# NVIDIA/flownet2-pytorch

Hardware: AMD Instinct MI355X
Metric: image-pairs/sec, FlowNet2 custom-layer hot path (Correlation + Resample2d + ChannelNorm) fwd+bwd @ 384x512 bs8 -- the whole FlowNet2C network's fwd+bwd image-pairs/sec is flownet2c.fwd_bwd_image_pairs_per_s; corr-layer HBM GB/s vs roofline is `roofline` (higher is better)
Workload: dtype f32; 1 GPU; FlowNet2 custom-layer hot path fwd+bwd, bs8 @384x512: Correlation 8x256x48x64 (20,1,20,1,2) [BASELINE configs[1]] + Resample2d 8x3x384x512 + ChannelNorm 8x3x384x512

## Files before the change

flownet2-pytorch_amd/csrc/corr_params.h:

```cpp
#pragma once
#include "fn2_common.h"

namespace fn2 {

struct CorrP {
    int B, C, H, W;
    int pad, k, md, s1, s2;
    int kr, dr, D, nOut, oH, oW;
    long out_bs;
    float slope;
};

int corr_make_params(CorrP &p, int B, int C, int H, int W, int pad, int k, int md, int s1, int s2);
int corr_forward_direct(const void *in1, const void *in2, void *out, int dtype, const CorrP &p, hipStream_t s);
int corr_backward_direct(const void *in1, const void *in2, const void *gout, void *g1, void *g2, int dtype,
                         const CorrP &p, hipStream_t s);

bool corr_dense_applicable(int dtype, int C, int H, int W, int pad, int k, int md, int s1, int s2);
bool corr_dense_forward_pays(const CorrP &p);
int corr_forward_dense(const void *in1, const void *in2, void *out, int dtype, const CorrP &p, hipStream_t s);
int corr_backward_dense(const void *in1, const void *in2, const void *gout, void *g1, void *g2, int dtype,
                        const CorrP &p, hipStream_t s);
bool corr_mfma_f32_applicable(int dtype, int C, int H, int W, int pad, int k, int md, int s1, int s2);
int corr_forward_mfma_f32(const float *in1, const float *in2, float *out, long out_bs, float slope, int B, int C, int H,
                          int W, int md, int tune, hipStream_t s);

bool corr_f16x2_applicable(int dtype, int C, int H, int W, int pad, int k, int md, int s1, int s2);
int corr_forward_f16x2(const float *in1, const float *in2, float *out, long out_bs, float slope, int B, int C, int H, int W,
                       int variant, hipStream_t s);
int corr_forward_f16x2_wide(const float *in1, const float *in2, float *out, long out_bs, float slope, int B, int C, int H, int W,
                            hipStream_t s);

bool corr_f16_fwd_applicable(int dtype, int C, int H, int W, int pad, int k, int md, int s1, int s2);
int corr_forward_f16(int dtype, const void *in1, const void *in2, void *out, long out_bs, float slope, int B, int C, int H, int W,
                     hipStream_t s);

bool corr_f16_bwd_applicable(int dtype, int C, int H, int W, int pad, int k, int md, int s1, int s2);
int corr_backward_f16(int dtype, const void *in1, const void *in2, const void *gout, void *g1, void *g2, int B, int C, int H, int W,
                      hipStream_t s);

void corr_f16x2_set_debug_buffer(void *p);
void *corr_f16x2_get_debug_buffer();
bool corr_bwd_f16x2_applicable(int dtype, int C, int H, int W, int pad, int k, int md, int s1, int s2);
int corr_backward_f16x2(const float *in1, const float *in2, const float *gout, float *g1, float *g2, int B, int C, int H, int W,
                        int variant, hipStream_t s);
int corr_backward_f16x2_wide(const float *in1, const float *in2, const float *gout, float *g1, float *g2, int B, int C, int H, int W,
                             hipStream_t s);

bool corr_bwd_mfma_f32_applicable(int dtype, int C, int H, int W, int pad, int k, int md, int s1, int s2);
int corr_backward_mfma_f32(const float *in1, const float *in2, const float *gout, float *g1, float *g2,
                           int B, int C, int H, int W, int md, int tune, hipStream_t s);

bool corr_mfma_f64_applicable(int dtype, int C, int H, int W, int pad, int k, int md, int s1, int s2);
int corr_forward_mfma_f64(const double *in1, const double *in2, double *out, long out_bs, double slope, int B, int C, int H, int W, hipStream_t s);
int corr_backward_mfma_f64(const double *in1, const double *in2, const double *gout, double *g1, double *g2, int B, int C, int H, int W, hipStream_t s);

}
```

flownet2-pytorch_amd/csrc/correlation_f16_bwd.hip:

```cpp
#include <type_traits>

#include "corr_params.h"

#ifndef FN2_HBH_ABL
#define FN2_HBH_ABL 0
#endif

namespace fn2 {
namespace hbh {
constexpr int ABL = FN2_HBH_ABL;

typedef float f4 __attribute__((ext_vector_type(4)));
typedef unsigned u4 __attribute__((ext_vector_type(4)));
typedef unsigned u2 __attribute__((ext_vector_type(2)));
#define FN2_LDS(T) __attribute__((address_space(3))) T

constexpr int DR = 10, D = 21, NU = 6;
constexpr int CG = 64, NCT = CG / 16;
constexpr int CK = 32;
constexpr int CHS = 288, PARS = CK * CHS, XBUF = 2 * PARS;
template <int FLIP> struct GL {
    static constexpr int BI = 256;
    static constexpr int TI = FLIP ? 1024 + 4 : 1024 + 32;
    static constexpr int AI = FLIP ? D * TI + 76 : D * TI + 128;
// ... 61 lines not shown
struct XSet { u4 v[XK]; };
struct GSet { u4 v[NGL]; };

template <class E>
__global__ __launch_bounds__(NWAVES * 64, 3) void corr_bwd_f16(Args<E> p)
{
    typedef typename Op16<E>::v8 h8;
    __shared__ __attribute__((aligned(16))) char smem[LDS_BYTES];

    const int tid = threadIdx.x, lane = tid & 63;
    const int wave = __builtin_amdgcn_readfirstlane(tid >> 6);
    const bool is_stage = wave < NSW;
    const int w8 = is_stage ? wave : wave - NSW;
    const int HL = p.H >> 1;
    const int hw = p.H * p.W;
    const long HW = (long)p.H * p.W;
    const int per_fn = 2 * p.NRG * p.NCGR;
    const int ntasks = 2 * p.B * per_fn;
    const bool pow2 = (p.C & (p.C - 1)) == 0;

    struct Task { int flip, n, py, rg, cg; };
    auto get_task = [&](int t) -> Task {
        Task k;
        k.cg = t % p.NCGR; t /= p.NCGR;
        k.rg = t % p.NRG; t /= p.NRG;
        k.py = t & 1; t >>= 1;
        k.n = t % p.B;
        k.flip = t / p.B;
        k.cg = __builtin_amdgcn_readfirstlane(k.cg); k.rg = __builtin_amdgcn_readfirstlane(k.rg);
        k.py = __builtin_amdgcn_readfirstlane(k.py); k.n = __builtin_amdgcn_readfirstlane(k.n);
        k.flip = __builtin_amdgcn_readfirstlane(k.flip);
        return k;
    };

    float *Es = reinterpret_cast<float *>(smem + X_OFS);
    auto store_rows = [&](const Task &tk) {
        if (ABL & 32) return;
        int ln = lane;
        asm volatile("" : "+v"(ln));
        const int g = ln >> 4, xg = 4 * (ln & 15);
        constexpr int NRI = (CG + NWAVES - 1) / NWAVES;
        const int y = 2 * (4 * tk.rg + g) + tk.py;
        const bool lane_ok = 4 * tk.rg + g < HL && xg < p.W;
        const unsigned vo = lane_ok ? (unsigned)((y * p.W + xg) * 2) : 0x80000000u;
        const __amdgpu_buffer_rsrc_t rso = __builtin_amdgcn_make_buffer_rsrc(p.gin[tk.flip] + (long)tk.n * p.C * HW, 0, (unsigned)(p.C * hw * 2), 0x00020000);
        auto chan = [&](int i) { return wave + NWAVES * i; };
        auto read_row = [&](int c) {
            return *reinterpret_cast<const f4 *>(Es + (c * 4 + g) * 64 + ((xg + 8 * g + 32 * ((c >> 2) & 1)) & 63));
        };
        f4 vals[NRI];
#pragma unroll
        for (int i = 0; i < NRI; ++i) vals[i] = read_row(chan(i) & (CG - 1));
        float r, f = 1.0f;
        asm volatile("v_mov_b32 %0, %1" : "=v"(r) : "s"(p.rC));
        if (!pow2) asm volatile("v_mov_b32 %0, %1" : "=v"(f) : "s"(p.fC));
        auto finish = [&](f4 val) -> u2 {
            if (pow2) { val[0] *= r; val[1] *= r; val[2] *= r; val[3] *= r; }
            else { val[0] /= f; val[1] /= f; val[2] /= f; val[3] /= f; }
            return (u2){Op16<E>::pk(val[0], val[1]), Op16<E>::pk(val[2], val[3])};
        };
        unsigned bad = 0;
#pragma unroll
        for (int i = 0; i < NRI; ++i) {
            const int c = chan(i);
            if (c >= CG) continue;
            if (lane_ok && (__builtin_amdgcn_classf(vals[i][0], 0x207) | __builtin_amdgcn_classf(vals[i][1], 0x207) |
// ... 73 lines not shown
            asm volatile("" : "+v"(ln));
            const int ts = ln >> 3, pc = ln & 7;
            if (tk.flip) {
                char *dst = smem + w8 * GL<1>::AI + ts * GL<1>::TI + pc * 32;
#pragma unroll
                for (int i = 0; i < NGL; ++i) {
                    const int bi = i / 3, tb = i % 3;
                    if (tb == 2 && ts + 16 >= D) continue;
                    const h8 h = __builtin_bit_cast(h8, S.v[i]);
                    FN2_LDS(float) *d = (FN2_LDS(float) *)(dst + 8 * tb * GL<1>::TI + bi * 256);
#pragma unroll
                    for (int e = 0; e < 8; ++e) d[e] = (float)h[e];
                }
            } else {
                char *dst = smem + w8 * GL<0>::AI + ts * GL<0>::TI + pc * 32;
#pragma unroll
                for (int i = 0; i < NGL; ++i) {
                    const int bi = i / 3, tb = i % 3;
                    if (tb == 2 && ts + 16 >= D) continue;
                    const h8 h = __builtin_bit_cast(h8, S.v[i]);
                    *(FN2_LDS(f4) *)(dst + 8 * tb * GL<0>::TI + bi * 256) = (f4){(float)h[0], (float)h[1], (float)h[2], (float)h[3]};
                    *(FN2_LDS(f4) *)(dst + 8 * tb * GL<0>::TI + bi * 256 + 16) = (f4){(float)h[4], (float)h[5], (float)h[6], (float)h[7]};
                }
            }
        };
        auto pick = [](bool c, const Task &a, const Task &b) {
            Task r;
            r.flip = c ? a.flip : b.flip; r.n = c ? a.n : b.n; r.py = c ? a.py : b.py; r.rg = c ? a.rg : b.rg; r.cg = c ? a.cg : b.cg;
            return r;
        };
        XSet XA0, XA1, XB0, XB1;
        GSet GS;
        int t = (int)xcd_remap(blockIdx.x, gridDim.x);
        if (t < ntasks) {
            const Task tk = get_task(t);
            g_issue(GS, tk, 0, true);
            x_issue(XA0, tk, 0, 0, true);
            x_issue(XA1, tk, 0, 1, true);
            g_write(GS, tk);
            g_issue(GS, tk, 1, true);
        }
        __syncthreads();
        for (; t < ntasks; t += gridDim.x) {
            const Task tk = get_task(t);
            const bool has_next = t + (int)gridDim.x < ntasks;
            const Task tn = get_task(has_next ? t + (int)gridDim.x : t);
            auto one_u = [&](int u, XSet &C0, XSet &C1, XSet &N0, XSet &N1) {
                const bool more = u + 1 < NU, more2 = u + 2 < NU;
                const Task t1 = pick(more, tk, tn), t2 = pick(more2, tk, tn);
                x_issue(N0, t1, more ? u + 1 : 0, 0, more || has_next);
                x_issue(N1, t1, more ? u + 1 : 0, 1, more || has_next);
                x_write(C0, smem + X_OFS);
                x_write(C1, smem + X_OFS + XBUF);
                __syncthreads();
                if (more || has_next) g_write(GS, t1);
                g_issue(GS, t2, more2 ? u + 2 : u + 2 - NU, more2 || has_next);
                __syncthreads();
            };
            for (int u = 0; u < NU; u += 2) {
                one_u(u, XA0, XA1, XB0, XB1);
                one_u(u + 1, XB0, XB1, XA0, XA1);
            }
            __syncthreads();
            store_rows(tk);
            __syncthreads();
        }
        return;
    }

    const int xpar = w8 & 1;
    const int role = __builtin_amdgcn_readfirstlane(w8 >> 1);

    auto run_task = [&](const Task &tk, auto flipc) {
        constexpr int FLIP = decltype(flipc)::value;
        int ln = lane;
        asm volatile("" : "+v"(ln));
        const int f_i = ln & 15, f_g = ln >> 4;
        const int f_ai = f_i >> 2, f_aj = f_i & 3;
        const int xb = xpar * PARS + f_i * CHS + f_g * 16;

        f4 acc[2][NCT];
#pragma unroll
        for (int ab = 0; ab < 2; ++ab)
#pragma unroll
            for (int ct = 0; ct < NCT; ++ct) acc[ab][ct] = (f4){0.0f, 0.0f, 0.0f, 0.0f};
        h8 gh[NF];

        auto gather = [&](auto role_c, auto xp_c) {
            constexpr int R = decltype(role_c)::value;
            constexpr int XP = decltype(xp_c)::value;
            typedef GL<FLIP> L;
            constexpr int SB = L::TI - 8;
            int l2 = lane;
            asm volatile("" : "+v"(l2));
// ... 46 lines not shown
#pragma unroll
                    for (int ct = 0; ct < NCT; ++ct)
                        x[ct] = *reinterpret_cast<const h8 *>(smem + X_OFS + (ct >> 1) * XBUF + xb + (ct & 1) * 16 * CHS + j * 64);
                    if (ABL & 1) { asm volatile("" ::"v"(x[0]), "v"(x[1]), "v"(x[2]), "v"(x[3])); return; }
#pragma unroll
                    for (int ct = 0; ct < NCT; ++ct) {
                        if constexpr (f0 >= 0) acc[0][ct] = Op16<E>::mfma(x[ct], gh[f0 >= 0 ? f0 : 0], acc[0][ct]);
                        if constexpr (f1 >= 0) acc[1][ct] = Op16<E>::mfma(x[ct], gh[f1 >= 0 ? f1 : 0], acc[1][ct]);
                    }
                    __builtin_amdgcn_sched_barrier(0);
                }
            });
        };
        auto gather_d = [&]() {
            auto by_role = [&](auto xp_c) {
                switch (role) {
                case 0: gather(std::integral_constant<int, 0>{}, xp_c); break;
                case 1: gather(std::integral_constant<int, 1>{}, xp_c); break;
                case 2: gather(std::integral_constant<int, 2>{}, xp_c); break;
                default: gather(std::integral_constant<int, 3>{}, xp_c); break;
                }
            };
            if (xpar) by_role(std::integral_constant<int, 1>{});
            else by_role(std::integral_constant<int, 0>{});
        };
        auto mma_d = [&]() {
            switch (role) {
            case 0: mma(std::integral_constant<int, 0>{}); break;
            case 1: mma(std::integral_constant<int, 1>{}); break;
            case 2: mma(std::integral_constant<int, 2>{}); break;
            default: mma(std::integral_constant<int, 3>{}); break;
            }
        };
        for (int u = 0; u < NU; ++u) {
            gather_d();
            __syncthreads();
            mma_d();
            __syncthreads();
        }
        auto scatter = [&](auto role_c) {
            constexpr int R = decltype(role_c)::value;
            static_for<0, 2>([&](auto abc) {
                constexpr int ab = decltype(abc)::value;
                constexpr int a = a_blk(R, ab);
                const int x = 8 * a + 2 * f_aj + xpar;
                static_for<0, NCT>([&](auto ctc) {
                    constexpr int ct = decltype(ctc)::value;
                    static_for<0, 4>([&](auto rc) {
                        constexpr int r = decltype(rc)::value;
                        const int c = 16 * ct + 4 * f_g + r;
                        Es[(c * 4 + f_ai) * 64 + ((x + 8 * f_ai + 32 * (f_g & 1)) & 63)] = acc[ab][ct][r];
                    });
                });
            });
        };
        if (ABL & 32) {
#pragma unroll
            for (int ab = 0; ab < 2; ++ab)
#pragma unroll
                for (int ct = 0; ct < NCT; ++ct) asm volatile("" ::"v"(acc[ab][ct]));
        } else {
            switch (role) {
            case 0: scatter(std::integral_constant<int, 0>{}); break;
            case 1: scatter(std::integral_constant<int, 1>{}); break;
            case 2: scatter(std::integral_constant<int, 2>{}); break;
            default: scatter(std::integral_constant<int, 3>{}); break;
            }
// ... 52 lines not shown
```

flownet2-pytorch_amd/csrc/correlation_f16x2_bwd.hip:

```cpp
#include <type_traits>

#include "corr_params.h"
#include "f16x2_split.h"

namespace fn2 {
namespace hb {
using f16s::exp_stat;
using f16s::scale_exp;
using f16s::split2;
using f16s::to_sgpr;
using f16s::wave_sum;

typedef float f4 __attribute__((ext_vector_type(4)));
typedef float f2 __attribute__((ext_vector_type(2)));
typedef _Float16 h2 __attribute__((ext_vector_type(2)));
typedef _Float16 h8 __attribute__((ext_vector_type(8)));
typedef short s8 __attribute__((ext_vector_type(8)));
typedef unsigned u4 __attribute__((ext_vector_type(4)));
typedef unsigned u2 __attribute__((ext_vector_type(2)));
#define FN2_LDS(T) __attribute__((address_space(3))) T

#ifdef FN2_ABL_BWDTEMPORAL
constexpr int BWD_STORE_AUX = 0;
#else
// ... 93 lines not shown
    asm volatile("v_mbcnt_lo_u32_b32 %0, -1, 0\n\tv_mbcnt_hi_u32_b32 %0, -1, %0" : "=v"(l));
    return l;
}

template <int VAR>
__global__ __launch_bounds__(NWAVES * 64, 3) void corr_bwd_f16x2(Args p)
{
    __shared__ __attribute__((aligned(16))) char smem[LDS_BYTES];
    __shared__ int scl_k[2];
    __shared__ __attribute__((aligned(16))) float scl_sx[2][CG];

    const int tid = threadIdx.x, lane = tid & 63;
    const int wave = __builtin_amdgcn_readfirstlane(tid >> 6);
    const bool is_stage = wave < NSW;
    const int w8 = is_stage ? wave : wave - NSW;
    const int HL = p.H >> 1;
    const long HW = (long)p.H * p.W;
    const int per_fn = 2 * p.NRG * p.NCGR;
    const int ntasks = p.nflip * p.B * per_fn;
    const bool pow2 = (p.C & (p.C - 1)) == 0;
    const int lgC = pow2 ? 31 - __builtin_clz((unsigned)p.C) : 0;
    if (tid < 16) reinterpret_cast<unsigned *>(smem + ZERO_OFS)[tid] = 0u;
    unsigned long long ts[16];
#pragma unroll
    for (int i = 0; i < 16; ++i) ts[i] = 0;
    auto stamp = [&](int i) __attribute__((always_inline)) { if (VAR & 64) ts[i] = __builtin_amdgcn_s_memtime(); };
    auto dump = [&]() __attribute__((always_inline)) {
        if ((VAR & 64) && p.dbg && lane == 0 && (wave == 0 || wave == NSW)) {
            unsigned long long *d = p.dbg + (blockIdx.x * 2 + (wave ? 1 : 0)) * 16;
#pragma unroll
            for (int i = 0; i < 16; ++i) d[i] = ts[i];
        }
    };
    stamp(0);

    struct Task { int flip, n, py, rg, cg; };
    auto get_task = [&](int t) -> Task {
        Task k;
        k.cg = t % p.NCGR; t /= p.NCGR;
        k.rg = t % p.NRG; t /= p.NRG;
#ifdef FN2_ABL_FLIPOUTER
        k.py = t & 1; t >>= 1;
        k.n = t % p.B;
        k.flip = p.nflip == 2 ? t / p.B : p.flip0;
#else
        k.flip = p.nflip == 2 ? t % 2 : p.flip0;
        if (p.nflip == 2) t >>= 1;
        k.py = t & 1; t >>= 1;
        k.n = t;
#endif
        k.cg = __builtin_amdgcn_readfirstlane(k.cg); k.rg = __builtin_amdgcn_readfirstlane(k.rg);
        k.py = __builtin_amdgcn_readfirstlane(k.py); k.n = __builtin_amdgcn_readfirstlane(k.n);
        k.flip = __builtin_amdgcn_readfirstlane(k.flip);
        return k;
    };

    float *Es = reinterpret_cast<float *>(smem + X_OFS);
    auto store_rows = [&](const Task &tk, int kg, int par) {
        int ln = lane_now();
        const int g = ln >> 4, xg = 4 * (ln & 15);
        constexpr int NRI = (CG + NWAVES - 1) / NWAVES;
        const int y = 2 * (4 * tk.rg + g) + tk.py;
        const bool lane_ok = 4 * tk.rg + g < HL && xg < p.W;
        const unsigned vo = lane_ok ? (unsigned)((y * p.W + xg) * 4) : 0x80000000u;
        const __amdgpu_buffer_rsrc_t rso = __builtin_amdgcn_make_buffer_rsrc(p.gin[tk.flip] + (long)tk.n * p.C * HW, 0, (unsigned)(p.C * HW * 4), 0x00020000);
        auto chan = [&](int i) { return wave + NWAVES * i; };
        auto read_row = [&](int c) {
            return *reinterpret_cast<const f4 *>(Es + (c * 4 + g) * 64 + ((xg + 8 * g + 32 * ((c >> 2) & 1)) & 63));
        };
        f4 vals[NRI];
#pragma unroll
        for (int i = 0; i < NRI; ++i) vals[i] = read_row(chan(i) & (CG - 1));
        float f = 1.0f;
        if (!pow2) asm volatile("v_mov_b32 %0, %1" : "=v"(f) : "s"(p.fC));
        const int kx_ex = -lgC;
        auto ksum_of = [&](int c) {
            const int cc = c & (CG - 1);
            const int bits = to_sgpr(__builtin_bit_cast(int, scl_sx[par][8 * (cc & 7) + (cc >> 3)]));
            return (bits >> 23) - 127 + kg;
        };
        auto scaled = [&](f4 val, int kx) {
#pragma unroll
            for (int e = 0; e < 4; ++e) val[e] = __builtin_ldexpf(val[e], kx);
            if (!pow2) { val[0] /= f; val[1] /= f; val[2] /= f; val[3] /= f; }
            return val;
        };
        unsigned bad = 0;
// ... 101 lines not shown
            const int tj = tk.flip ? 20 - 4 * U0 - bi + ai : 4 * U0 + bi - ai;
            const int ilg = tk.flip ? 4 * tk.rg - DR + 4 * U0 + bi : 4 * tk.rg + ai;
            const int x = 2 * (((((5 * ln) >> 1) & 31) * (p.W >> 1)) >> 5);
            const int c = tk.cg * CG + ln, ilx = min(4 * tk.rg + (ln & 3), HL - 1);
            const int ti = (5 * q + (ln & 3) + bi) % D;
            const unsigned ox = (ilx >= 0 && ilx < HL) ? (unsigned)((c * HW + (long)(2 * ilx + tk.py) * p.W + x) * 4) : 0x80000000u;
            const int ilx2 = min(4 * tk.rg + ((ln + 2) & 3), HL - 1), xb = (x + (p.W >> 1)) >= p.W ? x + (p.W >> 1) - p.W : x + (p.W >> 1);
            const unsigned ox2 = (ilx2 >= 0 && ilx2 < HL) ? (unsigned)((c * HW + (long)(2 * ilx2 + tk.py) * p.W + xb) * 4) : 0x80000000u;
            const unsigned og = (ilg >= 0 && ilg < HL) ? (unsigned)((((tj * D + ti) * p.H + 2 * ilg + tk.py) * p.W + x) * 4) : 0x80000000u;
#ifdef FN2_ABL_NOSAMPLELOAD
            S.x = (u2)0x3f000000u; S.x2 = S.x; S.g = (u2)0x3f000000u; (void)ox; (void)ox2; (void)og;
#else
            S.x = (VAR & 2) ? (u2)0x3f800000u : __builtin_amdgcn_raw_buffer_load_b64(rsx, (int)ox, 0, 0);
            S.x2 = (VAR & 2) ? (u2)0x3f800000u : __builtin_amdgcn_raw_buffer_load_b64(rsx, (int)ox2, 0, 0);
            S.g = (VAR & 2) ? (u2)0x3f800000u : __builtin_amdgcn_raw_buffer_load_b64(rsg, (int)og, 0, 0);
#endif
        };
        auto sample_scales = [&](const Samp &S, int &kx, int &kg) {
            const unsigned t4 = exp_stat(S.x[0]) + exp_stat(S.x[1]) + exp_stat(S.x2[0]) + exp_stat(S.x2[1]);
            const unsigned sum = t4 & 0xffffu, cnt = t4 >> 16;
            const int em = cnt ? (int)((2u * sum + cnt) / (2u * cnt)) : 0;
            const int k = f16s::T_GEO + 127 - em;
            kx = cnt == 0u ? 0 : (k < -126 ? -126 : k > 127 ? 127 : k);
            const unsigned tg = exp_stat(S.g[0]) + exp_stat(S.g[1]);
            kg = scale_exp(wave_sum(tg));
        };
        auto publish = [&](int par, int kx, int kg) {
            if (wave == 0) {
                int ln = lane_now();
                scl_sx[par][8 * (ln & 7) + (ln >> 3)] = f16s::scale_from_exp(kx);
                if (ln == 0) scl_k[1] = kg;
            }
        };
        XSet XA0, XA1, XB0, XB1;
        int t = (int)xcd_remap(blockIdx.x, gridDim.x);
        Samp SM;
        int kx_n = 0, kg_n = 0;
        int it = 0;
        if (t < ntasks) {
            const Task tk = get_task(t);
            sample_issue(tk, SM);
            x_issue(XA0, tk, 0, 0);
            x_issue(XA1, tk, 0, 1);
            g_dma(tk, 0);
            stamp(1);
            dma_wait();
            stamp(2);
            sample_scales(SM, kx_n, kg_n);
            publish(0, kx_n, kg_n);
        }
        __syncthreads();
        stamp(3);
        for (; t < ntasks; t += gridDim.x) {
            const Task tk = get_task(t);
            const bool has_next = t + (int)gridDim.x < ntasks;
            const Task tn = get_task(has_next ? t + (int)gridDim.x : t);
            const bool first = t < (int)gridDim.x;
            const int kg_cur = kg_n, par = it & 1;
            auto one_u = [&](int u, XSet &C0, XSet &C1, XSet &N0, XSet &N1) {
                const float *sxp = &scl_sx[par][8 * s_ch];
                float sc = sxp[0];
                if (u + 1 < NU) { x_issue(N0, tk, u + 1, 0); x_issue(N1, tk, u + 1, 1); }
                else if (has_next) { x_issue(N0, tn, 0, 0); x_issue(N1, tn, 0, 1); }
#pragma unroll
                for (int k = 0; k < 2 * XK; ++k) {
                    const float nx = sxp[k + 1 < 2 * XK ? k + 1 : k];
                    if (k < XK) x_write1(C0, smem + X_OFS, k, sc);
                    else x_write1(C1, smem + X_OFS + XBUF, k - XK, sc);
                    sc = nx;
                }
                if (first && u < 2) stamp(4 + 4 * u);
                __syncthreads();
                if (first && u < 2) stamp(5 + 4 * u);
                if (u + 1 < NU) g_dma(tk, u + 1);
                else if (has_next) { sample_issue(tn, SM); g_dma(tn, 0); }
                dma_wait();
                if (first && u < 2) stamp(6 + 4 * u);
                __syncthreads();
                if (first && u < 2) stamp(7 + 4 * u);
            };
            for (int u = 0; u < NU; u += 2) {
                one_u(u, XA0, XA1, XB0, XB1);
                one_u(u + 1, XB0, XB1, XA0, XA1);
            }
            if (has_next) { sample_scales(SM, kx_n, kg_n); publish(par ^ 1, kx_n, kg_n); }
            if (first) stamp(12);
            __syncthreads();
            if (first) stamp(13);
            store_rows(tk, kg_cur, par);
            __syncthreads();
            if (first) stamp(14);
            ++it;
        }
        stamp(15);
        dump();
        return;
    }

    if (VAR & 256) __builtin_amdgcn_s_setprio(2);
    const int xpar = w8 & 1;
    const int role = __builtin_amdgcn_readfirstlane(w8 >> 1);

    int itm = 0;
    auto run_task = [&](const Task &tk, auto flipc, bool first) {
        constexpr int FLIP = decltype(flipc)::value;
        const int kg_cur = to_sgpr(scl_k[1]);
        const f16s::scale2_t sc_g2 = f16s::scale2_from_exp(kg_cur);
        int ln = lane_now();
        const int f_i = ln & 15, f_g = ln >> 4;
        const int f_ai = f_i >> 2, f_aj = f_i & 3;
        const int xb = xpar * PARS + f_i * CHS + f_g * 16;

        f4 acc[2][NCT];
#pragma unroll
        for (int ab = 0; ab < 2; ++ab)
#pragma unroll
            for (int ct = 0; ct < NCT; ++ct) acc[ab][ct] = (f4){0.0f, 0.0f, 0.0f, 0.0f};
        h8 gh[NF], gl[NF];

        auto gather = [&](auto role_c, auto xp_c) {
            constexpr int R = decltype(role_c)::value;
            constexpr int XP = decltype(xp_c)::value;
            typedef GL<FLIP> L;
            constexpr int SB = L::TI - 8;
            int l2 = lane_now();
            const int ai = (l2 & 15) >> 2, aj = l2 & 3, blk = (l2 >> 4) & 1, gg = l2 >> 5;
            const int lbase = FLIP ? ai * L::AI + 2 * gg * L::BI + (DR - 4 * blk + aj) * L::TI - 3 * SB + 32 * blk + 4 * XP
                                   : ai * L::AI + 2 * gg * L::BI + (DR + 4 * blk - aj) * L::TI + 8 * aj;
            const int vs = 4 * blk - aj;
            static_for<0, 2>([&](auto abc) {
                constexpr int ab = decltype(abc)::value;
                constexpr int a = a_blk(R, ab);
                static_for<0, 4>([&](auto jc) {
                    constexpr int j = decltype(jc)::value;
                    constexpr int fi = frag_idx(R, ab, j);
                    if constexpr (fi >= 0) {
// ... 75 lines not shown
                                    if constexpr (f0 >= 0)
                                        acc[0][2 * ch + c2] = __builtin_amdgcn_mfma_f32_16x16x32_f16(pr == 2 ? xl[c2] : xh[c2], pr == 1 ? gl[f0 >= 0 ? f0 : 0] : gh[f0 >= 0 ? f0 : 0], acc[0][2 * ch + c2], 0, 0, 0);
                                    if constexpr (f1 >= 0)
                                        acc[1][2 * ch + c2] = __builtin_amdgcn_mfma_f32_16x16x32_f16(pr == 2 ? xl[c2] : xh[c2], pr == 1 ? gl[f1 >= 0 ? f1 : 0] : gh[f1 >= 0 ? f1 : 0], acc[1][2 * ch + c2], 0, 0, 0);
                                }
                            });
                        }
                        __builtin_amdgcn_sched_barrier(0);
                    });
                }
            });
        };
        auto gather_x = [&](auto xp_c) {
            switch (role) {
            case 0: gather(std::integral_constant<int, 0>{}, xp_c); break;
            case 1: gather(std::integral_constant<int, 1>{}, xp_c); break;
            case 2: gather(std::integral_constant<int, 2>{}, xp_c); break;
            default: gather(std::integral_constant<int, 3>{}, xp_c); break;
            }
        };
        auto gather_d = [&]() {
            if (xpar) gather_x(std::integral_constant<int, 1>{});
            else gather_x(std::integral_constant<int, 0>{});
        };
        auto mma_d = [&]() {
            switch (role) {
            case 0: mma(std::integral_constant<int, 0>{}); break;
            case 1: mma(std::integral_constant<int, 1>{}); break;
            case 2: mma(std::integral_constant<int, 2>{}); break;
            default: mma(std::integral_constant<int, 3>{}); break;
            }
        };

        for (int u = 0; u < NU; ++u) {
            gather_d();
            if (first && u < 2) stamp(4 + 4 * u);
            __syncthreads();
            if (first && u < 2) stamp(5 + 4 * u);
            mma_d();
            if (first && u < 2) stamp(6 + 4 * u);
            __syncthreads();
            if (first && u < 2) stamp(7 + 4 * u);
        }
        if (first) stamp(12);

        auto scatter = [&](auto role_c) {
            constexpr int R = decltype(role_c)::value;
            static_for<0, 2>([&](auto abc) {
                constexpr int ab = decltype(abc)::value;
                constexpr int a = a_blk(R, ab);
                const int x = 8 * a + 2 * f_aj + xpar;
                static_for<0, NCT>([&](auto ctc) {
                    constexpr int ct = decltype(ctc)::value;
                    static_for<0, 4>([&](auto rc) {
                        constexpr int r = decltype(rc)::value;
                        const int c = 16 * ct + 4 * f_g + r;
                        Es[(c * 4 + f_ai) * 64 + ((x + 8 * f_ai + 32 * (f_g & 1)) & 63)] = acc[ab][ct][r];
                    });
                });
            });
        };
        switch (role) {
        case 0: scatter(std::integral_constant<int, 0>{}); break;
        case 1: scatter(std::integral_constant<int, 1>{}); break;
        case 2: scatter(std::integral_constant<int, 2>{}); break;
        default: scatter(std::integral_constant<int, 3>{}); break;
        }
        __syncthreads();
        if (first) stamp(13);
        store_rows(tk, kg_cur, itm & 1);
        __syncthreads();
        if (first) stamp(14);
    };
    __syncthreads();
    stamp(3);
    for (int t = (int)xcd_remap(blockIdx.x, gridDim.x); t < ntasks; t += gridDim.x, ++itm) {
        const Task tk = get_task(t);
        const bool first = t < (int)gridDim.x;
        if (tk.flip) run_task(tk, std::integral_constant<int, 1>{}, first);
        else run_task(tk, std::integral_constant<int, 0>{}, first);
    }
    stamp(15);
    dump();
}

}

bool corr_bwd_f16x2_applicable(int dtype, int C, int H, int W, int pad, int k, int md, int s1, int s2)
{
    if (dtype != FN2_F32) return false;
    if (k != 1 || s1 != 1 || s2 != 2 || pad != md || md != 2 * hb::DR) return false;
    if (C % hb::CG != 0 || C < hb::CG || (H & 1) || (W % 8) != 0) return false;
    if ((long)C * H * W * 4 >= 0x7fffffffL || (long)hb::D * hb::D * H * W * 4 >= 0x7fffffffL) return false;
    return true;
}

int corr_backward_f16x2(const float *in1, const float *in2, const float *gout, float *g1, float *g2, int B, int C, int H, int W,
                        int variant, hipStream_t s)
{
    if (!aligned(in1, 16) || !aligned(in2, 16) || !aligned(gout, 16) || !aligned(g1, 16) || !aligned(g2, 16)) return FN2_EALIGN;
    if (W > 64) return variant == 0 ? corr_backward_f16x2_wide(in1, in2, gout, g1, g2, B, C, H, W, s) : FN2_EINVAL;
    hb::Args a;
    a.nbr[0] = in2; a.nbr[1] = in1; a.gout = gout; a.gin[0] = g1; a.gin[1] = g2;
    a.B = B; a.C = C; a.H = H; a.W = W;
    a.NRG = (H / 2 + 3) / 4; a.NCGR = C / hb::CG;
    a.nflip = 2; a.flip0 = 0;
    a.fC = (float)C; a.rC = 1.0f / (float)C;
#ifdef FN2_DEBUG_BUILD
    a.dbg = (variant & 64) ? static_cast<unsigned long long *>(corr_f16x2_get_debug_buffer()) : nullptr;
#else
    a.dbg = nullptr;
#endif
    const long ntasks = 2L * B * 2 * a.NRG * a.NCGR;
    if (ntasks == 0) return FN2_OK;
    if (ntasks > 0x3fffffffL) return FN2_EINVAL;
// ... 14 lines not shown
```

flownet2-pytorch_amd/csrc/correlation_f16x2_bwd_wide.hip:

```cpp
#include <type_traits>

#include "corr_params.h"
#include "f16x2_split.h"

namespace fn2 {
namespace hbw {
using f16s::exp_stat;
using f16s::scale_exp;
using f16s::split2;
using f16s::to_sgpr;
using f16s::wave_sum;

typedef float f4 __attribute__((ext_vector_type(4)));
typedef float f2 __attribute__((ext_vector_type(2)));
typedef _Float16 h8 __attribute__((ext_vector_type(8)));
typedef unsigned u4 __attribute__((ext_vector_type(4)));
typedef unsigned u2 __attribute__((ext_vector_type(2)));
#define FN2_LDS(T) __attribute__((address_space(3))) T

constexpr int DR = 10, D = 21, NU = 6;
constexpr int CG = 64, NCT = CG / 16;
constexpr int CK = 32;
constexpr int CHS = 288, PARS = CK * CHS, XTERM = 2 * PARS, XBUF = 2 * XTERM;
template <int FLIP> struct GL {
// ... 67 lines not shown
        }
    return s;
}

constexpr int NSW = 4, NWAVES = NSW + 8;
constexpr int XK = 32 / (2 * NSW);
struct XSet { u4 v[XK][2]; };

__device__ __forceinline__ int lane_now()
{
    int l;
    asm volatile("v_mbcnt_lo_u32_b32 %0, -1, 0\n\tv_mbcnt_hi_u32_b32 %0, -1, %0" : "=v"(l));
    return l;
}

__global__ __launch_bounds__(NWAVES * 64, 3) void corr_bwd_f16x2_wide(Args p)
{
    __shared__ __attribute__((aligned(16))) char smem[LDS_BYTES];
    __shared__ int scl_k[2];
    __shared__ __attribute__((aligned(16))) float scl_sx[2][CG];

    const int tid = threadIdx.x, lane = tid & 63;
    const int wave = __builtin_amdgcn_readfirstlane(tid >> 6);
    const bool is_stage = wave < NSW;
    const int w8 = is_stage ? wave : wave - NSW;
    const int HL = p.H >> 1;
    const long HW = (long)p.H * p.W;
    const int hw = p.H * p.W;
    const int per_fn = 2 * p.NRG * p.NXW * p.NCGR;
    const int ntasks = 2 * p.B * per_fn;
    const bool pow2 = (p.C & (p.C - 1)) == 0;
    const int lgC = pow2 ? 31 - __builtin_clz((unsigned)p.C) : 0;

    struct Task { int flip, n, py, rg, xw, cg, nv; };
    auto get_task = [&](int t) -> Task {
        Task k;
        k.cg = t % p.NCGR; t /= p.NCGR;
        k.xw = t % p.NXW; t /= p.NXW;
        k.rg = t % p.NRG; t /= p.NRG;
        k.py = t & 1; t >>= 1;
        k.n = t % p.B;
        k.flip = t / p.B;
        k.cg = __builtin_amdgcn_readfirstlane(k.cg); k.rg = __builtin_amdgcn_readfirstlane(k.rg);
        k.xw = __builtin_amdgcn_readfirstlane(k.xw);
        k.py = __builtin_amdgcn_readfirstlane(k.py); k.n = __builtin_amdgcn_readfirstlane(k.n);
        k.flip = __builtin_amdgcn_readfirstlane(k.flip);
        k.nv = (WPX * k.xw + 8 * PO(1) < p.W) ? 2 * NU : NU;
        return k;
    };
    auto nbr_x0 = [&](const Task &tk, int v) { return WPX * tk.xw + 8 * (v >= NU ? PO(1) : PO(0)); };

    float *Es = reinterpret_cast<float *>(smem + X_OFS);
    auto store_rows = [&](const Task &tk, int kg, int par) {
        int ln = lane_now();
        const int g = ln >> 4, xg = 4 * (ln & 15), xw = WPX * tk.xw + xg;
        constexpr int NRI = (CG + NWAVES - 1) / NWAVES;
        const int y = 2 * (4 * tk.rg + g) + tk.py;
        const bool lane_ok = 4 * tk.rg + g < HL && xw < p.W;
        const unsigned vo = lane_ok ? (unsigned)((y * p.W + xw) * 4) : 0x80000000u;
        const __amdgpu_buffer_rsrc_t rso = __builtin_amdgcn_make_buffer_rsrc(p.gin[tk.flip] + (long)tk.n * p.C * HW, 0, (unsigned)(p.C * HW * 4), 0x00020000);
        auto chan = [&](int i) { return wave + NWAVES * i; };
        auto read_row = [&](int c) {
            return *reinterpret_cast<const f4 *>(Es + (c * 4 + g) * 64 + ((xg + 8 * g + 32 * ((c >> 2) & 1)) & 63));
        };
        f4 vals[NRI];
#pragma unroll
        for (int i = 0; i < NRI; ++i) vals[i] = read_row(chan(i) & (CG - 1));
        float f = 1.0f;
        if (!pow2) asm volatile("v_mov_b32 %0, %1" : "=v"(f) : "s"(p.fC));
        const int kx_ex = -lgC;
        auto ksum_of = [&](int c) {
            const int cc = c & (CG - 1);
            const int bits = to_sgpr(__builtin_bit_cast(int, scl_sx[par][8 * (cc & 7) + (cc >> 3)]));
            return (bits >> 23) - 127 + kg;
        };
        auto scaled = [&](f4 val, int kx) {
#pragma unroll
            for (int e = 0; e < 4; ++e) val[e] = __builtin_ldexpf(val[e], kx);
            if (!pow2) { val[0] /= f; val[1] /= f; val[2] /= f; val[3] /= f; }
            return val;
        };
        unsigned bad = 0;
// ... 87 lines not shown
            const __amdgpu_buffer_rsrc_t rsx = __builtin_amdgcn_make_buffer_rsrc(const_cast<float *>(p.nbr[tk.flip] + (long)tk.n * p.C * HW), 0, xbytes, 0x00020000);
            const __amdgpu_buffer_rsrc_t rsg = __builtin_amdgcn_make_buffer_rsrc(const_cast<float *>(p.gout + (long)tk.n * D * D * HW), 0, gbytes, 0x00020000);
            const int ai = ln & 3, bi = (ln >> 2) & 3, q = ln >> 4;
            const int tj = tk.flip ? 20 - 4 * U0 - bi + ai : 4 * U0 + bi - ai;
            const int ilg = tk.flip ? 4 * tk.rg - DR + 4 * U0 + bi : 4 * tk.rg + ai;
            const int xs = 2 * (((5 * ln) >> 1) & 31), xs2 = (xs + 32) & 63;
            const int x = WPX * tk.xw + (WPX * tk.xw + xs < p.W ? xs : xs & 7);
            const int c = tk.cg * CG + ln, ilx = min(4 * tk.rg + (ln & 3), HL - 1);
            const int ti = (5 * q + (ln & 3) + bi) % D;
            const unsigned ox = (ilx >= 0 && ilx < HL && x < p.W) ? (unsigned)((c * HW + (long)(2 * ilx + tk.py) * p.W + x) * 4) : 0x80000000u;
            const int ilx2 = min(4 * tk.rg + ((ln + 2) & 3), HL - 1), xb = WPX * tk.xw + (WPX * tk.xw + xs2 < p.W ? xs2 : xs2 & 7);
            const unsigned ox2 = (ilx2 >= 0 && ilx2 < HL && xb < p.W) ? (unsigned)((c * HW + (long)(2 * ilx2 + tk.py) * p.W + xb) * 4) : 0x80000000u;
            const unsigned og = (ilg >= 0 && ilg < HL && x < p.W) ? (unsigned)((((tj * D + ti) * p.H + 2 * ilg + tk.py) * p.W + x) * 4) : 0x80000000u;
            S.x = __builtin_amdgcn_raw_buffer_load_b64(rsx, (int)ox, 0, 0);
            S.x2 = __builtin_amdgcn_raw_buffer_load_b64(rsx, (int)ox2, 0, 0);
            S.g = __builtin_amdgcn_raw_buffer_load_b64(rsg, (int)og, 0, 0);
        };
        auto sample_scales = [&](const Samp &S, int &kx, int &kg) {
            const unsigned t4 = exp_stat(S.x[0]) + exp_stat(S.x[1]) + exp_stat(S.x2[0]) + exp_stat(S.x2[1]);
            const unsigned sum = t4 & 0xffffu, cnt = t4 >> 16;
            const int em = cnt ? (int)((2u * sum + cnt) / (2u * cnt)) : 0;
            const int k = f16s::T_GEO + 127 - em;
            kx = cnt == 0u ? 0 : (k < -126 ? -126 : k > 127 ? 127 : k);
            const unsigned tg = exp_stat(S.g[0]) + exp_stat(S.g[1]);
            kg = scale_exp(wave_sum(tg));
        };
        auto publish = [&](int par, int kx, int kg) {
            if (wave == 0) {
                int ln = lane_now();
                scl_sx[par][8 * (ln & 7) + (ln >> 3)] = f16s::scale_from_exp(kx);
                if (ln == 0) scl_k[1] = kg;
            }
        };
        XSet XA0, XA1, XB0, XB1;
        int t = (int)xcd_remap(blockIdx.x, gridDim.x);
        Samp SM;
        int kx_n = 0, kg_n = 0;
        int it = 0;
        if (t < ntasks) {
            const Task tk = get_task(t);
            sample_issue(tk, SM);
            x_issue(XA0, tk, 0, 0);
            x_issue(XA1, tk, 0, 1);
            g_dma(tk, 0);
            dma_wait();
            sample_scales(SM, kx_n, kg_n);
            publish(0, kx_n, kg_n);
        }
        __syncthreads();
        for (; t < ntasks; t += gridDim.x) {
            const Task tk = get_task(t);
            const bool has_next = t + (int)gridDim.x < ntasks;
            const Task tn = get_task(has_next ? t + (int)gridDim.x : t);
            const int kg_cur = kg_n, par = it & 1;
            auto one_v = [&](int v, XSet &C0, XSet &C1, XSet &N0, XSet &N1) {
                int l5 = lane_now();
                const float *sxp = &scl_sx[par][8 * (2 * w8 + (l5 >> 5))];
                float sc = sxp[0];
                if (v + 1 < tk.nv) { x_issue(N0, tk, v + 1, 0); x_issue(N1, tk, v + 1, 1); }
                else if (has_next) { x_issue(N0, tn, 0, 0); x_issue(N1, tn, 0, 1); }
                const int w_ofs = x_ofs();
#pragma unroll
                for (int k = 0; k < 2 * XK; ++k) {
                    const float nx = sxp[k + 1 < 2 * XK ? k + 1 : k];
                    if (k < XK) x_write1(C0, smem + X_OFS, w_ofs, k, sc);
                    else x_write1(C1, smem + X_OFS + XBUF, w_ofs, k - XK, sc);
                    sc = nx;
                }
                __syncthreads();
                if (v + 1 < tk.nv) g_dma(tk, v + 1);
                else if (has_next) { sample_issue(tn, SM); g_dma(tn, 0); }
                dma_wait();
                __syncthreads();
            };
            for (int v = 0; v < tk.nv; v += 2) {
                one_v(v, XA0, XA1, XB0, XB1);
                one_v(v + 1, XB0, XB1, XA0, XA1);
            }
            if (has_next) { sample_scales(SM, kx_n, kg_n); publish(par ^ 1, kx_n, kg_n); }
            __syncthreads();
            store_rows(tk, kg_cur, par);
            __syncthreads();
            ++it;
        }
        return;
    }

    const int xpar = w8 & 1;
    const int role = __builtin_amdgcn_readfirstlane(w8 >> 1);

    int itm = 0;
    auto run_task = [&](const Task &tk, auto flipc) {
        constexpr int FLIP = decltype(flipc)::value;
        const int kg_cur = to_sgpr(scl_k[1]);
        const f16s::scale2_t sc_g2 = f16s::scale2_from_exp(kg_cur);
        int ln = lane_now();
        const int f_i = ln & 15, f_g = ln >> 4;
        const int f_ai = f_i >> 2, f_aj = f_i & 3;
        const int xb = xpar * PARS + f_i * CHS + f_g * 16;

        f4 acc[2][NCT];
#pragma unroll
        for (int ab = 0; ab < 2; ++ab)
#pragma unroll
            for (int ct = 0; ct < NCT; ++ct) acc[ab][ct] = (f4){0.0f, 0.0f, 0.0f, 0.0f};
        h8 gh[NF], gl[NF];

        auto gather = [&](auto ps_c, auto role_c, auto xp_c) {
            constexpr int PS = decltype(ps_c)::value;
            constexpr int R = decltype(role_c)::value;
// ... 70 lines not shown
                            for (int c2 = 0; c2 < 2; ++c2) {
                                if constexpr (f0 >= 0)
                                    acc[0][2 * ch + c2] = __builtin_amdgcn_mfma_f32_16x16x32_f16(pr == 2 ? xl[c2] : xh[c2], pr == 1 ? gl[f0 >= 0 ? f0 : 0] : gh[f0 >= 0 ? f0 : 0], acc[0][2 * ch + c2], 0, 0, 0);
                                if constexpr (f1 >= 0)
                                    acc[1][2 * ch + c2] = __builtin_amdgcn_mfma_f32_16x16x32_f16(pr == 2 ? xl[c2] : xh[c2], pr == 1 ? gl[f1 >= 0 ? f1 : 0] : gh[f1 >= 0 ? f1 : 0], acc[1][2 * ch + c2], 0, 0, 0);
                            }
                        });
                        __builtin_amdgcn_sched_barrier(0);
                    });
                }
            });
        };
        auto gather_d = [&](auto ps_c) {
            auto by_role = [&](auto xp_c) {
                switch (role) {
                case 0: gather(ps_c, std::integral_constant<int, 0>{}, xp_c); break;
                case 1: gather(ps_c, std::integral_constant<int, 1>{}, xp_c); break;
                case 2: gather(ps_c, std::integral_constant<int, 2>{}, xp_c); break;
                default: gather(ps_c, std::integral_constant<int, 3>{}, xp_c); break;
                }
            };
            if (xpar) by_role(std::integral_constant<int, 1>{});
            else by_role(std::integral_constant<int, 0>{});
        };
        auto mma_d = [&](auto ps_c) {
            switch (role) {
            case 0: mma(ps_c, std::integral_constant<int, 0>{}); break;
            case 1: mma(ps_c, std::integral_constant<int, 1>{}); break;
            case 2: mma(ps_c, std::integral_constant<int, 2>{}); break;
            default: mma(ps_c, std::integral_constant<int, 3>{}); break;
            }
        };
        auto one_pass = [&](auto ps_c) {
            for (int u = 0; u < NU; ++u) {
                gather_d(ps_c);
                __syncthreads();
                mma_d(ps_c);
                __syncthreads();
            }
        };
        one_pass(std::integral_constant<int, 0>{});
        if (tk.nv > NU) one_pass(std::integral_constant<int, 1>{});

        auto scatter = [&](auto role_c) {
            constexpr int R = decltype(role_c)::value;
            static_for<0, 2>([&](auto abc) {
                constexpr int ab = decltype(abc)::value;
                constexpr int a = a_blk(R, ab);
                const int x = 8 * a + 2 * f_aj + xpar;
                static_for<0, NCT>([&](auto ctc) {
                    constexpr int ct = decltype(ctc)::value;
                    static_for<0, 4>([&](auto rc) {
                        constexpr int r = decltype(rc)::value;
                        const int c = 16 * ct + 4 * f_g + r;
                        Es[(c * 4 + f_ai) * 64 + ((x + 8 * f_ai + 32 * (f_g & 1)) & 63)] = acc[ab][ct][r];
                    });
                });
            });
        };
        switch (role) {
        case 0: scatter(std::integral_constant<int, 0>{}); break;
        case 1: scatter(std::integral_constant<int, 1>{}); break;
        case 2: scatter(std::integral_constant<int, 2>{}); break;
        default: scatter(std::integral_constant<int, 3>{}); break;
        }
        __syncthreads();
        store_rows(tk, kg_cur, itm & 1);
        __syncthreads();
    };
    __syncthreads();
    for (int t = (int)xcd_remap(blockIdx.x, gridDim.x); t < ntasks; t += gridDim.x, ++itm) {
        const Task tk = get_task(t);
        if (tk.flip) run_task(tk, std::integral_constant<int, 1>{});
        else run_task(tk, std::integral_constant<int, 0>{});
    }
// ... 23 lines not shown
```

Before: 43810 image-pairs/s.

## Skip out-of-range row blocks in correlation backward f16 kernels

After: 45760 image-pairs/s, median of 6. 1.04x the previous value.

```diff
diff --git a/flownet2-pytorch_amd/csrc/corr_params.h b/flownet2-pytorch_amd/csrc/corr_params.h
--- a/flownet2-pytorch_amd/csrc/corr_params.h
+++ b/flownet2-pytorch_amd/csrc/corr_params.h
@@ -39,6 +39,15 @@
 int corr_backward_f16(int dtype, const void *in1, const void *in2, const void *gout, void *g1, void *g2, int B, int C, int H, int W,
                       hipStream_t s);
 
+struct URange { int lo, hi; };
+__host__ __device__ constexpr URange bwd_u_range(int rg, int HL, int dr = 10, int nu = 6)
+{
+    const int lo = (dr - 4 * rg) >> 2, hi = (HL - 1 + dr - 4 * rg) >> 2;
+    return URange{lo < 0 ? 0 : lo, hi > nu - 1 ? nu - 1 : hi};
+}
+static_assert(bwd_u_range(0, 24).lo == 2 && bwd_u_range(1, 24).lo == 1 && bwd_u_range(2, 24).lo == 0 && bwd_u_range(3, 24).hi == 5 &&
+              bwd_u_range(4, 24).hi == 4 && bwd_u_range(5, 24).hi == 3 && bwd_u_range(0, 1).lo == 2 && bwd_u_range(0, 1).hi == 2, "real row blocks");
+
 void corr_f16x2_set_debug_buffer(void *p);
 void *corr_f16x2_get_debug_buffer();
 bool corr_bwd_f16x2_applicable(int dtype, int C, int H, int W, int pad, int k, int md, int s1, int s2);
diff --git a/flownet2-pytorch_amd/csrc/correlation_f16_bwd.hip b/flownet2-pytorch_amd/csrc/correlation_f16_bwd.hip
--- a/flownet2-pytorch_amd/csrc/correlation_f16_bwd.hip
+++ b/flownet2-pytorch_amd/csrc/correlation_f16_bwd.hip
@@ -117,6 +117,7 @@
         k.flip = __builtin_amdgcn_readfirstlane(k.flip);
         return k;
     };
+    auto task_u = [&](const Task &k) -> URange { return bwd_u_range(k.rg, HL, DR, NU); };
 
     float *Es = reinterpret_cast<float *>(smem + X_OFS);
     auto store_rows = [&](const Task &tk) {
@@ -256,34 +257,51 @@
         XSet XA0, XA1, XB0, XB1;
         GSet GS;
         int t = (int)xcd_remap(blockIdx.x, gridDim.x);
+        const int gs = (int)gridDim.x;
         if (t < ntasks) {
             const Task tk = get_task(t);
-            g_issue(GS, tk, 0, true);
-            x_issue(XA0, tk, 0, 0, true);
-            x_issue(XA1, tk, 0, 1, true);
+            const URange ur = task_u(tk);
+            const bool more = ur.lo < ur.hi, has_next = t + gs < ntasks;
+            const Task t1 = more ? tk : get_task(has_next ? t + gs : t);
+            g_issue(GS, tk, ur.lo, true);
+            x_issue(XA0, tk, ur.lo, 0, true);
+            x_issue(XA1, tk, ur.lo, 1, true);
             g_write(GS, tk);
-            g_issue(GS, tk, 1, true);
+            g_issue(GS, t1, more ? ur.lo + 1 : task_u(t1).lo, more || has_next);
         }
         __syncthreads();
-        for (; t < ntasks; t += gridDim.x) {
+        for (; t < ntasks; t += gs) {
             const Task tk = get_task(t);
-            const bool has_next = t + (int)gridDim.x < ntasks;
-            const Task tn = get_task(has_next ? t + (int)gridDim.x : t);
-            auto one_u = [&](int u, XSet &C0, XSet &C1, XSet &N0, XSet &N1) {
-                const bool more = u + 1 < NU, more2 = u + 2 < NU;
-                const Task t1 = pick(more, tk, tn), t2 = pick(more2, tk, tn);
-                x_issue(N0, t1, more ? u + 1 : 0, 0, more || has_next);
-                x_issue(N1, t1, more ? u + 1 : 0, 1, more || has_next);
+            const bool has_next = t + gs < ntasks, has_next2 = t + 2 * gs < ntasks;
+            const Task tn = get_task(has_next ? t + gs : t);
+            const Task tnn = get_task(has_next2 ? t + 2 * gs : t);
+            const URange ur = task_u(tk), un = task_u(tn);
+            const int unn_lo = task_u(tnn).lo;
+            auto one_u = [&](int u, XSet &C0, XSet &C1, XSet &N0, XSet &N1) -> bool {
+                const bool more = u < ur.hi;
+                const Task t1 = pick(more, tk, tn);
+                const int u1 = more ? u + 1 : un.lo;
+                const bool v1 = more || has_next;
+                const bool more2 = more ? u + 1 < ur.hi : un.lo < un.hi;
+                const Task t2 = pick(more2, t1, pick(more, tn, tnn));
+                const int u2 = more2 ? u1 + 1 : (more ? un.lo : unn_lo);
+                const bool v2 = more2 ? v1 : (more ? has_next : has_next2);
+                x_issue(N0, t1, u1, 0, v1);
+                x_issue(N1, t1, u1, 1, v1);
                 x_write(C0, smem + X_OFS);
                 x_write(C1, smem + X_OFS + XBUF);
                 __syncthreads();
-                if (more || has_next) g_write(GS, t1);
-                g_issue(GS, t2, more2 ? u + 2 : u + 2 - NU, more2 || has_next);
+                if (v1) g_write(GS, t1);
+                g_issue(GS, t2, u2, v2);
                 __syncthreads();
+                return !more;
             };
-            for (int u = 0; u < NU; u += 2) {
-                one_u(u, XA0, XA1, XB0, XB1);
-                one_u(u + 1, XB0, XB1, XA0, XA1);
+            for (int u = ur.lo;; u += 2) {
+                if (one_u(u, XA0, XA1, XB0, XB1)) {
+                    XA0 = XB0; XA1 = XB1;
+                    break;
+                }
+                if (one_u(u + 1, XB0, XB1, XA0, XA1)) break;
             }
             __syncthreads();
             store_rows(tk);
@@ -396,7 +414,8 @@
             default: mma(std::integral_constant<int, 3>{}); break;
             }
         };
-        for (int u = 0; u < NU; ++u) {
+        const URange ur = task_u(tk);
+        for (int u = ur.lo; u <= ur.hi; ++u) {
             gather_d();
             __syncthreads();
             mma_d();
diff --git a/flownet2-pytorch_amd/csrc/correlation_f16x2_bwd.hip b/flownet2-pytorch_amd/csrc/correlation_f16x2_bwd.hip
--- a/flownet2-pytorch_amd/csrc/correlation_f16x2_bwd.hip
+++ b/flownet2-pytorch_amd/csrc/correlation_f16x2_bwd.hip
@@ -149,6 +149,10 @@
             for (int i = 0; i < 16; ++i) d[i] = ts[i];
         }
     };
+    auto stamp_u = [&](int si, int k) __attribute__((always_inline)) {
+        if (si == 0) stamp(4 + k);
+        else if (si == 1) stamp(8 + k);
+    };
     stamp(0);
 
     struct Task { int flip, n, py, rg, cg; };
@@ -170,6 +174,13 @@
         k.py = __builtin_amdgcn_readfirstlane(k.py); k.n = __builtin_amdgcn_readfirstlane(k.n);
         k.flip = __builtin_amdgcn_readfirstlane(k.flip);
         return k;
+    };
+    auto task_u = [&](const Task &k) -> URange {
+        URange r = bwd_u_range(k.rg, HL, DR, NU);
+#ifdef FN2_ABL_EVENU
+        if (!((r.hi - r.lo) & 1)) { if (r.lo > 0) --r.lo; else ++r.hi; }
+#endif
+        return r;
     };
 
     float *Es = reinterpret_cast<float *>(smem + X_OFS);
@@ -337,6 +348,11 @@
                 if (ln == 0) scl_k[1] = kg;
             }
         };
+        auto pick = [](bool c, const Task &a, const Task &b) {
+            Task r;
+            r.flip = c ? a.flip : b.flip; r.n = c ? a.n : b.n; r.py = c ? a.py : b.py; r.rg = c ? a.rg : b.rg; r.cg = c ? a.cg : b.cg;
+            return r;
+        };
         XSet XA0, XA1, XB0, XB1;
         int t = (int)xcd_remap(blockIdx.x, gridDim.x);
         Samp SM;
@@ -344,10 +360,11 @@
         int it = 0;
         if (t < ntasks) {
             const Task tk = get_task(t);
+            const int u0 = task_u(tk).lo;
             sample_issue(tk, SM);
-            x_issue(XA0, tk, 0, 0);
-            x_issue(XA1, tk, 0, 1);
-            g_dma(tk, 0);
+            x_issue(XA0, tk, u0, 0);
+            x_issue(XA1, tk, u0, 1);
+            g_dma(tk, u0);
             stamp(1);
             dma_wait();
             stamp(2);
@@ -362,11 +379,16 @@
             const Task tn = get_task(has_next ? t + (int)gridDim.x : t);
             const bool first = t < (int)gridDim.x;
             const int kg_cur = kg_n, par = it & 1;
-            auto one_u = [&](int u, XSet &C0, XSet &C1, XSet &N0, XSet &N1) {
+            const URange ur = task_u(tk);
+            const int un_lo = task_u(tn).lo;
+            auto one_u = [&](int u, XSet &C0, XSet &C1, XSet &N0, XSet &N1) -> bool {
+                const bool last = u == ur.hi;
+                const Task t1 = pick(last, tn, tk);
+                const int u1 = last ? un_lo : u + 1;
+                const int si = u - ur.lo;
                 const float *sxp = &scl_sx[par][8 * s_ch];
                 float sc = sxp[0];
-                if (u + 1 < NU) { x_issue(N0, tk, u + 1, 0); x_issue(N1, tk, u + 1, 1); }
-                else if (has_next) { x_issue(N0, tn, 0, 0); x_issue(N1, tn, 0, 1); }
+                x_issue(N0, t1, u1, 0); x_issue(N1, t1, u1, 1);
 #pragma unroll
                 for (int k = 0; k < 2 * XK; ++k) {
                     const float nx = sxp[k + 1 < 2 * XK ? k + 1 : k];
@@ -374,19 +396,23 @@
                     else x_write1(C1, smem + X_OFS + XBUF, k - XK, sc);
                     sc = nx;
                 }
-                if (first && u < 2) stamp(4 + 4 * u);
+                if (first) stamp_u(si, 0);
                 __syncthreads();
-                if (first && u < 2) stamp(5 + 4 * u);
-                if (u + 1 < NU) g_dma(tk, u + 1);
-                else if (has_next) { sample_issue(tn, SM); g_dma(tn, 0); }
+                if (first) stamp_u(si, 1);
+                if (last && has_next) sample_issue(tn, SM);
+                if (!last || has_next) g_dma(t1, u1);
                 dma_wait();
-                if (first && u < 2) stamp(6 + 4 * u);
+                if (first) stamp_u(si, 2);
                 __syncthreads();
-                if (first && u < 2) stamp(7 + 4 * u);
+                if (first) stamp_u(si, 3);
+                return last;
             };
-            for (int u = 0; u < NU; u += 2) {
-                one_u(u, XA0, XA1, XB0, XB1);
-                one_u(u + 1, XB0, XB1, XA0, XA1);
+            for (int u = ur.lo;; u += 2) {
+                if (one_u(u, XA0, XA1, XB0, XB1)) {
+                    XA0 = XB0; XA1 = XB1;
+                    break;
+                }
+                if (one_u(u + 1, XB0, XB1, XA0, XA1)) break;
             }
             if (has_next) { sample_scales(SM, kx_n, kg_n); publish(par ^ 1, kx_n, kg_n); }
             if (first) stamp(12);
@@ -407,6 +433,7 @@
     const int role = __builtin_amdgcn_readfirstlane(w8 >> 1);
 
     int itm = 0;
+    int steps_run = 0;
     auto run_task = [&](const Task &tk, auto flipc, bool first) {
         constexpr int FLIP = decltype(flipc)::value;
         const int kg_cur = to_sgpr(scl_k[1]);
@@ -548,16 +575,19 @@
             }
         };
 
-        for (int u = 0; u < NU; ++u) {
+        const URange ur = task_u(tk);
+        const int nsteps = ur.hi - ur.lo + 1;
+        for (int si = 0; si < nsteps; ++si) {
             gather_d();
-            if (first && u < 2) stamp(4 + 4 * u);
+            if (first) stamp_u(si, 0);
             __syncthreads();
-            if (first && u < 2) stamp(5 + 4 * u);
+            if (first) stamp_u(si, 1);
             mma_d();
-            if (first && u < 2) stamp(6 + 4 * u);
+            if (first) stamp_u(si, 2);
             __syncthreads();
-            if (first && u < 2) stamp(7 + 4 * u);
-        }
+            if (first) stamp_u(si, 3);
+        }
+        if (VAR & 64) steps_run += nsteps;
         if (first) stamp(12);
 
         auto scatter = [&](auto role_c) {
@@ -597,6 +627,7 @@
         else run_task(tk, std::integral_constant<int, 0>{}, first);
     }
     stamp(15);
+    if (VAR & 64) ts[1] = (unsigned long long)steps_run;
     dump();
 }
 
diff --git a/flownet2-pytorch_amd/csrc/correlation_f16x2_bwd_wide.hip b/flownet2-pytorch_amd/csrc/correlation_f16x2_bwd_wide.hip
--- a/flownet2-pytorch_amd/csrc/correlation_f16x2_bwd_wide.hip
+++ b/flownet2-pytorch_amd/csrc/correlation_f16x2_bwd_wide.hip
@@ -123,7 +123,7 @@
     const bool pow2 = (p.C & (p.C - 1)) == 0;
     const int lgC = pow2 ? 31 - __builtin_clz((unsigned)p.C) : 0;
 
-    struct Task { int flip, n, py, rg, xw, cg, nv; };
+    struct Task { int flip, n, py, rg, xw, cg, nv, ulo, cnt; };
     auto get_task = [&](int t) -> Task {
         Task k;
         k.cg = t % p.NCGR; t /= p.NCGR;
@@ -136,9 +136,12 @@
         k.xw = __builtin_amdgcn_readfirstlane(k.xw);
         k.py = __builtin_amdgcn_readfirstlane(k.py); k.n = __builtin_amdgcn_readfirstlane(k.n);
         k.flip = __builtin_amdgcn_readfirstlane(k.flip);
-        k.nv = (WPX * k.xw + 8 * PO(1) < p.W) ? 2 * NU : NU;
+        const URange ur = bwd_u_range(k.rg, HL, DR, NU);
+        k.ulo = ur.lo; k.cnt = ur.hi - ur.lo + 1;
+        k.nv = (WPX * k.xw + 8 * PO(1) < p.W) ? 2 * k.cnt : k.cnt;
         return k;
     };
+    auto v_of = [&](const Task &k, int s) { return s >= k.cnt ? NU + k.ulo + s - k.cnt : k.ulo + s; };
     auto nbr_x0 = [&](const Task &tk, int v) { return WPX * tk.xw + 8 * (v >= NU ? PO(1) : PO(0)); };
 
     float *Es = reinterpret_cast<float *>(smem + X_OFS);
@@ -292,6 +295,12 @@
                 if (ln == 0) scl_k[1] = kg;
             }
         };
+        auto pick = [](bool c, const Task &a, const Task &b) {
+            Task r;
+            r.flip = c ? a.flip : b.flip; r.n = c ? a.n : b.n; r.py = c ? a.py : b.py; r.rg = c ? a.rg : b.rg; r.xw = c ? a.xw : b.xw;
+            r.cg = c ? a.cg : b.cg; r.nv = c ? a.nv : b.nv; r.ulo = c ? a.ulo : b.ulo; r.cnt = c ? a.cnt : b.cnt;
+            return r;
+        };
         XSet XA0, XA1, XB0, XB1;
         int t = (int)xcd_remap(blockIdx.x, gridDim.x);
         Samp SM;
@@ -300,9 +309,9 @@
         if (t < ntasks) {
             const Task tk = get_task(t);
             sample_issue(tk, SM);
-            x_issue(XA0, tk, 0, 0);
-            x_issue(XA1, tk, 0, 1);
-            g_dma(tk, 0);
+            x_issue(XA0, tk, tk.ulo, 0);
+            x_issue(XA1, tk, tk.ulo, 1);
+            g_dma(tk, tk.ulo);
             dma_wait();
             sample_scales(SM, kx_n, kg_n);
             publish(0, kx_n, kg_n);
@@ -313,12 +322,14 @@
             const bool has_next = t + (int)gridDim.x < ntasks;
             const Task tn = get_task(has_next ? t + (int)gridDim.x : t);
             const int kg_cur = kg_n, par = it & 1;
-            auto one_v = [&](int v, XSet &C0, XSet &C1, XSet &N0, XSet &N1) {
+            auto one_v = [&](int s, XSet &C0, XSet &C1, XSet &N0, XSet &N1) -> bool {
+                const bool last = s + 1 == tk.nv;
+                const Task t1 = pick(last, tn, tk);
+                const int v1 = last ? tn.ulo : v_of(tk, s + 1);
                 int l5 = lane_now();
                 const float *sxp = &scl_sx[par][8 * (2 * w8 + (l5 >> 5))];
                 float sc = sxp[0];
-                if (v + 1 < tk.nv) { x_issue(N0, tk, v + 1, 0); x_issue(N1, tk, v + 1, 1); }
-                else if (has_next) { x_issue(N0, tn, 0, 0); x_issue(N1, tn, 0, 1); }
+                x_issue(N0, t1, v1, 0); x_issue(N1, t1, v1, 1);
                 const int w_ofs = x_ofs();
 #pragma unroll
                 for (int k = 0; k < 2 * XK; ++k) {
@@ -328,14 +339,18 @@
                     sc = nx;
                 }
                 __syncthreads();
-                if (v + 1 < tk.nv) g_dma(tk, v + 1);
-                else if (has_next) { sample_issue(tn, SM); g_dma(tn, 0); }
+                if (last && has_next) sample_issue(tn, SM);
+                if (!last || has_next) g_dma(t1, v1);
                 dma_wait();
                 __syncthreads();
+                return last;
             };
-            for (int v = 0; v < tk.nv; v += 2) {
-                one_v(v, XA0, XA1, XB0, XB1);
-                one_v(v + 1, XB0, XB1, XA0, XA1);
+            for (int s = 0;; s += 2) {
+                if (one_v(s, XA0, XA1, XB0, XB1)) {
+                    XA0 = XB0; XA1 = XB1;
+                    break;
+                }
+                if (one_v(s + 1, XB0, XB1, XA0, XA1)) break;
             }
             if (has_next) { sample_scales(SM, kx_n, kg_n); publish(par ^ 1, kx_n, kg_n); }
             __syncthreads();
@@ -472,7 +487,7 @@
             }
         };
         auto one_pass = [&](auto ps_c) {
-            for (int u = 0; u < NU; ++u) {
+            for (int u = 0; u < tk.cnt; ++u) {
                 gather_d(ps_c);
                 __syncthreads();
                 mma_d(ps_c);
@@ -480,7 +495,7 @@
             }
         };
         one_pass(std::integral_constant<int, 0>{});
-        if (tk.nv > NU) one_pass(std::integral_constant<int, 1>{});
+        if (tk.nv > tk.cnt) one_pass(std::integral_constant<int, 1>{});
 
         auto scatter = [&](auto role_c) {
             constexpr int R = decltype(role_c)::value;
```
